# jiali-ms/JLM

Measured on AMD Instinct MI355X. Metric: decoded chars/sec at beam=10, vocab=50k (kana strings in -> n-best strings out, SURVEY 8d), higher is better.
Workload: dtype f32 (matrix products as 3-pass split-f16 MFMA, f32 accumulate; the vocabulary projection as f16 hi.hi + both cross terms in one block-scaled FP6 instruction per 32 k-values: f32-grade error, tests/test_gpu_kernels.py; scores f64; parity bars: step logits <= 1e-4 relative, 1-best identical, path scor

## Files before the change

jlm_amd/csrc/jlm_beam.hip:

```cpp
#include "jlm_common.h"
#include <type_traits>
#include <stdlib.h>

#define WL_THREADS 256
#define WL_ROWS 16

template <int MODE>
__global__ __launch_bounds__(WL_THREADS) void wordlist_kernel(
    SegTable segs, const float *__restrict__ b2, const float *__restrict__ T, int ldt,
    const int *__restrict__ g0v, const int *__restrict__ cnt, const int *__restrict__ cnt_idx,
    const int *__restrict__ wl, const int *__restrict__ wl_w, const int *__restrict__ wl_off, const int *__restrict__ wl_idx,
    int wl_base, const int *__restrict__ wl_out, float *__restrict__ edge, float *__restrict__ run_max,
    double *__restrict__ run_sum, double *__restrict__ lse, int merge, int beam) {
    extern __shared__ __attribute__((aligned(16))) float sm[];
    const int j = blockIdx.x;
    const int nrows = min(cnt[cnt_idx[j]], beam);
    if (nrows <= 0) return;
    const int gbase = g0v[j];
    const int lid = wl_base + wl_idx[j];
    const int w0 = wl_off[lid], nw = wl_off[lid + 1] - w0;
    if (MODE == 0 && nw == 0) return;
    const int tid = threadIdx.x;
    float *red = sm + (size_t)WL_ROWS * ldt;
    const int sub = tid & 7, slot = tid >> 3;
// ... 191 lines not shown
                                     int merge, int beam, int n_groups, void *stream);

extern "C" int jlm_wordlist_lse(const jlm_segment *segs_host, int n_segs, const float *b2, const float *T, int ldt,
                                const int *g0, const int *cnt, const int *cnt_idx, const int *wl, const int *wl_off,
                                const int *wl_idx, int wl_base, float *run_max, double *run_sum, double *lse, int merge,
                                int beam, int n_groups, void *stream) {
    return jlm_wordlist_lse_perm(segs_host, n_segs, b2, T, ldt, g0, cnt, cnt_idx, wl, nullptr, wl_off, wl_idx, wl_base, run_max,
                                 run_sum, lse, merge, beam, n_groups, stream);
}

extern "C" int jlm_wordlist_lse_perm(const jlm_segment *segs_host, int n_segs, const float *b2, const float *T, int ldt,
                                     const int *g0, const int *cnt, const int *cnt_idx, const int *wl, const int *wl_w,
                                     const int *wl_off, const int *wl_idx, int wl_base, float *run_max, double *run_sum,
                                     double *lse, int merge, int beam, int n_groups, void *stream) {
    SegTable t;
    if (seg_table(segs_host, n_segs, t) || ldt % 4) return -1;
    if (n_groups <= 0) return 0;
    const int form = jlm_wordlist_lse_form(segs_host, n_segs, nullptr, wl_w != nullptr, ldt, beam, 0);
    if (form < 0) return -1;
    if (form == JLM_WL_MFMA)
        return jlm_wordlist_lse_mfma(segs_host, b2, T, ldt, g0, cnt, cnt_idx, wl, wl_off, wl_idx, wl_base, run_max, run_sum,
                                     lse, merge, beam, n_groups, stream);
    const size_t lds = wl_lds_bytes(beam, ldt);
    static JlmLdsGrant grant;
    if (int rc = jlm_grant_lds(grant, reinterpret_cast<const void *>(wordlist_kernel<1>), (int)lds)) return rc;
    hipLaunchKernelGGL(wordlist_kernel<1>, dim3(n_groups), dim3(WL_THREADS), lds, (hipStream_t)stream, t, b2, T, ldt,
                       g0, cnt, cnt_idx, wl, wl_w, wl_off, wl_idx, wl_base, nullptr, nullptr, run_max, run_sum, lse, merge, beam);
    JLM_LAUNCH_CHECK();
    return 0;
}

template <int CTRL, int ROW_MASK>
__device__ __forceinline__ void argmin_dpp_step(double &v, int &i) {
    const int lo = __double2loint(v), hi = __double2hiint(v);
    const int lo2 = __builtin_amdgcn_update_dpp(lo, lo, CTRL, ROW_MASK, 0xf, false);
    const int hi2 = __builtin_amdgcn_update_dpp(hi, hi, CTRL, ROW_MASK, 0xf, false);
    const int i2 = __builtin_amdgcn_update_dpp(i, i, CTRL, ROW_MASK, 0xf, false);
    const double v2 = __hiloint2double(hi2, lo2);
    if (v2 < v || (v2 == v && i2 < i)) { v = v2; i = i2; }
}
__device__ __forceinline__ void wave_argmin(double &v, int &i) {
    argmin_dpp_step<0xB1, 0xf>(v, i);
    argmin_dpp_step<0x4E, 0xf>(v, i);
    argmin_dpp_step<0x141, 0xf>(v, i);
    argmin_dpp_step<0x140, 0xf>(v, i);
    argmin_dpp_step<0x142, 0xa>(v, i);
    argmin_dpp_step<0x143, 0xc>(v, i);
    const int lo = __builtin_amdgcn_readlane(__double2loint(v), 63);
    const int hi = __builtin_amdgcn_readlane(__double2hiint(v), 63);
    i = __builtin_amdgcn_readlane(i, 63);
    v = __hiloint2double(hi, lo);
}

template <int MODE>
__global__ __launch_bounds__(64, 8) void beam_step_kernel(jlm_lattice lat, jlm_beam_state st, int frame, int max_cands) {
    extern __shared__ __attribute__((aligned(16))) double keys[];
    const int s = blockIdx.x, lane = threadIdx.x;
    const int B = lat.n_sent, beam = lat.beam, rmax = B * beam;
    const int len = lat.sent_len[s];
    const int fs = frame * B + s;
    if (frame > len) { if (lane == 0) st.cnt[fs] = 0; return; }
    const int nb = lat.end_off[fs], ne = lat.end_off[fs + 1];
    const int gout = frame * rmax + s * beam;
    const double INF = __longlong_as_double(0x7ff0000000000000LL);
    double *Sarr = keys + max_cands;
    int *gp_of = reinterpret_cast<int *>(Sarr + (MODE == 2 ? lat.n_frames * beam : 0));
    double *lse_new = reinterpret_cast<double *>(gp_of + ((max_cands + 1) & ~1));
    int *cnt_s = reinterpret_cast<int *>(lse_new + beam);
    double *win_v = reinterpret_cast<double *>(cnt_s + ((lat.n_frames + 1) & ~1));
    int *win_i = reinterpret_cast<int *>(win_v + beam);
    int K;
    if (frame == 0) {
        K = 1;
    } else {
        const bool fused = MODE == 0 && st.lse_part != nullptr;
        const int fprev = (frame - 1) * B + s;
        for (int f = lane; f < frame; f += 64) cnt_s[f] = st.cnt[f * B + s];
        const int kprev = st.cnt[fprev];
        if (fused && kprev > 0) {
            const int base = st.live_base[fprev];
            const float2 *part = reinterpret_cast<const float2 *>(st.lse_part);
            const int sub = lane & 7;
            for (int r0 = 0; r0 < kprev; r0 += 8) {
                const int r = r0 + (lane >> 3);
                float m = JLM_NEG_BIG;
                double sm = 0.0;
                if (r < kprev)
                    for (int p = sub; p < st.n_parts; p += 8) {
                        const float2 v = part[(size_t)p * st.ld_part + base + r];
                        const float mm = fmaxf(m, v.x);
                        sm = sm * (double)expf(m - mm) + (double)v.y * (double)expf(v.x - mm);
                        m = mm;
                    }
#pragma unroll
                for (int off = 4; off >= 1; off >>= 1) {
                    const float m2 = __shfl_xor(m, off);
                    const double s2 = __shfl_xor(sm, off);
                    const float mm = fmaxf(m, m2);
                    sm = sm * (double)expf(m - mm) + s2 * (double)expf(m2 - mm);
                    m = mm;
                }
                if (sub == 0 && r < kprev) {
                    double l = (double)m + log(sm);
                    if (!(fabs(l) < 1.0e300)) { if (st.flags) atomicOr(st.flags, 1); l = 1.0e30; }
                    lse_new[r] = l;
                    st.lse[(size_t)(frame - 1) * rmax + s * beam + r] = l;
                }
            }
        }
        const int C = (ne - nb) * beam;
        if (MODE == 2) {
            for (int f = 0; f < frame; ++f) {
                const int c = st.cnt[f * B + s];
                for (int l = lane; l < c; l += 64) {
                    const int g = f * rmax + s * beam + l;
                    const int p = st.bp[g];
                    double S = 0.0;
                    if (p >= 0) {
                        const int pf = p / rmax, pk = p - pf * rmax - s * beam;
                        S = Sarr[pf * beam + pk] + st.lse[p];
                    }
                    Sarr[f * beam + l] = S;
                }
                __syncthreads();
            }
        }
        __syncthreads();
        int nvalid = 0;
        double bv = INF;
        int bi = 0x7fffffff;
        constexpr int U = 4, NREG = 8;
        double kreg[NREG];
#pragma unroll
        for (int j = 0; j < NREG; ++j) kreg[j] = INF;
        auto group = [&](int it, auto REG0) {
            constexpr int reg0 = decltype(REG0)::value;
            const int c0 = lane + 64 * U * it;
            int n[U], k[U], sf[U];
#pragma unroll
            for (int u = 0; u < U; ++u) {
                const int c = min(c0 + 64 * u, C - 1);
                n[u] = nb + c / beam;
                k[u] = c % beam;
                sf[u] = lat.node_start[n[u]];
            }
            bool ok[U];
            double scv[U], lsv[U], ysv[U];
            float ev[U];
#pragma unroll
            for (int u = 0; u < U; ++u) {
                ok[u] = (c0 + 64 * u < C) && k[u] < cnt_s[sf[u]];
                const int gp = sf[u] * rmax + s * beam + (ok[u] ? k[u] : 0);
                ev[u] = st.edge[(size_t)n[u] * beam + k[u]];
                scv[u] = (MODE == 2) ? 0.0 : st.score[gp];
                lsv[u] = (MODE == 1) ? 0.0 : st.lse[gp];
                ysv[u] = (MODE == 2) ? st.ysum[gp] : 0.0;
                if (c0 + 64 * u < C) gp_of[c0 + 64 * u] = ok[u] ? gp : -1;
            }
#pragma unroll
            for (int u = 0; u < U; ++u) {
                const int c = c0 + 64 * u;
                if (c >= C) break;
                double sc = INF;
                if (ok[u]) {
                    const double e = (double)ev[u];
                    if (MODE == 0) sc = scv[u] + (((fused && sf[u] == frame - 1) ? lse_new[k[u]] : lsv[u]) - e);
                    else if (MODE == 1) sc = scv[u] - e;
                    else sc = (Sarr[sf[u] * beam + k[u]] + lsv[u]) - (ysv[u] + e);
                    ++nvalid;
                }
                if constexpr (reg0 >= 0) kreg[reg0 + u] = sc; else keys[c] = sc;
                if (sc < bv) { bv = sc; bi = c; }
            }
        };
        group(0, std::integral_constant<int, 0>{});
        if (C > 64 * U) group(1, std::integral_constant<int, U>{});
        for (int it = 2; 64 * U * it < C; ++it) group(it, std::integral_constant<int, -1>{});
#pragma unroll
        for (int off = 32; off >= 1; off >>= 1) nvalid += __shfl_xor(nvalid, off);
        K = min(beam, nvalid);
        for (int r = 0; r < K; ++r) {
            double v = bv;
            int i = bi;
            wave_argmin(v, i);
            if (lane == 0) { win_v[r] = v; win_i[r] = i; }
            if ((i & 63) == lane) {
                const int jw = i >> 6;
                if (jw >= NREG) keys[i] = INF;
                bv = INF;
                bi = 0x7fffffff;
#pragma unroll
                for (int j = 0; j < NREG; ++j) {
                    if (j == jw) kreg[j] = INF;
                    if (kreg[j] < bv) { bv = kreg[j]; bi = lane + 64 * j; }
                }
                for (int c = lane + 64 * NREG; c < C; c += 64) {
                    const double kv = keys[c];
                    if (kv < bv) { bv = kv; bi = c; }
                }
            }
        }
        __syncthreads();
    }
    for (int r = lane; r < K; r += 64) {
        const int g = gout + r;
        if (frame == 0) {
            st.score[g] = 0.0;
            if (st.ysum) st.ysum[g] = 0.0;
            st.bp[g] = -1;
            st.node[g] = nb;
            st.word[g] = lat.node_word[nb];
        } else {
            const int wi = win_i[r];
            const int n = nb + wi / beam, k = wi % beam;
            const int gp = gp_of[wi];
            st.score[g] = win_v[r];
            if (MODE == 2) st.ysum[g] = st.ysum[gp] + (double)st.edge[(size_t)n * beam + k];
            st.bp[g] = gp;
            st.node[g] = n;
            st.word[g] = lat.node_word[n];
        }
    }
    int base = 0;
    if (lane == 0) {
        st.cnt[fs] = K;
        if (frame < len) {
            base = atomicAdd(&st.n_live[frame], K);
            if (st.live_base) st.live_base[fs] = base;
        }
    }
    base = __shfl(base, 0);
    if (frame < len)
        for (int r = lane; r < K; r += 64) st.live[(size_t)frame * rmax + base + r] = gout + r;
}

template <int MODE>
__global__ __launch_bounds__(64) void beam_step_chunked_kernel(jlm_lattice lat, jlm_beam_state st, int frame, int cap, int nch_max) {
    extern __shared__ __attribute__((aligned(16))) double keys[];
    const int s = blockIdx.x, lane = threadIdx.x;
    const int B = lat.n_sent, beam = lat.beam, rmax = B * beam;
    const int len = lat.sent_len[s];
    const int fs = frame * B + s;
    if (frame > len) { if (lane == 0) st.cnt[fs] = 0; return; }
    const int nb = lat.end_off[fs], ne = lat.end_off[fs + 1];
    const int gout = frame * rmax + s * beam;
    const double INF = __longlong_as_double(0x7ff0000000000000LL);
    double *Sarr = keys + cap;
    int *gp_of = reinterpret_cast<int *>(Sarr + (MODE == 2 ? lat.n_frames * beam : 0));
    double *lse_new = reinterpret_cast<double *>(gp_of + ((cap + 1) & ~1));
    int *cnt_s = reinterpret_cast<int *>(lse_new + beam);
    double *win_v = reinterpret_cast<double *>(cnt_s + ((lat.n_frames + 1) & ~1));
    int *win_i = reinterpret_cast<int *>(win_v + beam);
    int *win_g = win_i + beam;
    double *cw_v = reinterpret_cast<double *>(win_g + beam + (beam & 1));
    int *cw_i = reinterpret_cast<int *>(cw_v + (size_t)nch_max * beam);
    int *cw_g = cw_i + (size_t)nch_max * beam;
    int K;
    if (frame == 0) {
        K = 1;
    } else {
        const bool fused = MODE == 0 && st.lse_part != nullptr;
        const int fprev = (frame - 1) * B + s;
        for (int f = lane; f < frame; f += 64) cnt_s[f] = st.cnt[f * B + s];
        const int kprev = st.cnt[fprev];
        if (fused && kprev > 0) {
            const int base = st.live_base[fprev];
            const float2 *part = reinterpret_cast<const float2 *>(st.lse_part);
            const int sub = lane & 7;
            for (int r0 = 0; r0 < kprev; r0 += 8) {
                const int r = r0 + (lane >> 3);
                float m = JLM_NEG_BIG;
                double sm = 0.0;
                if (r < kprev)
                    for (int p = sub; p < st.n_parts; p += 8) {
                        const float2 v = part[(size_t)p * st.ld_part + base + r];
                        const float mm = fmaxf(m, v.x);
                        sm = sm * (double)expf(m - mm) + (double)v.y * (double)expf(v.x - mm);
                        m = mm;
                    }
#pragma unroll
                for (int off = 4; off >= 1; off >>= 1) {
                    const float m2 = __shfl_xor(m, off);
                    const double s2 = __shfl_xor(sm, off);
                    const float mm = fmaxf(m, m2);
                    sm = sm * (double)expf(m - mm) + s2 * (double)expf(m2 - mm);
                    m = mm;
                }
                if (sub == 0 && r < kprev) {
                    double l = (double)m + log(sm);
                    if (!(fabs(l) < 1.0e300)) { if (st.flags) atomicOr(st.flags, 1); l = 1.0e30; }
                    lse_new[r] = l;
                    st.lse[(size_t)(frame - 1) * rmax + s * beam + r] = l;
                }
            }
        }
        const int C = (ne - nb) * beam;
        if (MODE == 2) {
            for (int f = 0; f < frame; ++f) {
                const int c = st.cnt[f * B + s];
                for (int l = lane; l < c; l += 64) {
                    const int g = f * rmax + s * beam + l;
                    const int p = st.bp[g];
                    double S = 0.0;
                    if (p >= 0) {
                        const int pf = p / rmax, pk = p - pf * rmax - s * beam;
                        S = Sarr[pf * beam + pk] + st.lse[p];
                    }
                    Sarr[f * beam + l] = S;
                }
                __syncthreads();
            }
        }
        __syncthreads();
        const int nch = (C + cap - 1) / cap;
        int nvalid_all = 0;
        for (int ch = 0; ch < nch; ++ch) {
            const int c_lo = ch * cap, Cc = min(C - c_lo, cap);
            int nvalid = 0;
            double bv = INF;
            int bi = 0x7fffffff;
            for (int lc = lane; lc < Cc; lc += 64) {
                const int c = c_lo + lc;
                const int n = nb + c / beam, k = c % beam;
                const int sf = lat.node_start[n];
                const bool ok = k < cnt_s[sf];
                const int gp = sf * rmax + s * beam + (ok ? k : 0);
                double sc = INF;
                if (ok) {
                    const double e = (double)st.edge[(size_t)n * beam + k];
                    if (MODE == 0) sc = st.score[gp] + (((fused && sf == frame - 1) ? lse_new[k] : st.lse[gp]) - e);
                    else if (MODE == 1) sc = st.score[gp] - e;
                    else sc = (Sarr[sf * beam + k] + st.lse[gp]) - (st.ysum[gp] + e);
                    ++nvalid;
                }
                keys[lc] = sc;
                gp_of[lc] = ok ? gp : -1;
                if (sc < bv) { bv = sc; bi = lc; }
            }
#pragma unroll
            for (int off = 32; off >= 1; off >>= 1) nvalid += __shfl_xor(nvalid, off);
            nvalid_all += nvalid;
            const int Kc = min(beam, nvalid);
            __syncthreads();
            for (int r = 0; r < beam; ++r) {
                if (r < Kc) {
                    double v = bv;
                    int i = bi;
                    wave_argmin(v, i);
// ... 117 lines not shown
}

struct BeamStepPlan { int form, cap, nch; size_t lds; };
static BeamStepPlan beam_step_plan(int beam, int n_frames, int mode, int max_cands) {
    BeamStepPlan p = {-1, 0, 0, 0};
    if (mode < 0 || mode > 2 || beam < 1 || beam > JLM_MAX_BEAM || n_frames < 1) return p;
    if (max_cands < 1) max_cands = 1;
    const size_t lds = beam_step_lds_bytes(beam, n_frames, mode, max_cands);
    static const int chunk_env = getenv("JLM_BEAM_CHUNK") ? atoi(getenv("JLM_BEAM_CHUNK")) : 0;
    if (lds > 160 * 1024 || chunk_env > 0) {
        const int cap = chunk_env > 0 ? chunk_env : beam_step_chunk_cap(beam, n_frames, mode);
        if (cap <= 0) return p;
        const int nch = (max_cands + cap - 1) / cap;
        const size_t lds_c = beam_step_chunked_lds_bytes(beam, n_frames, mode, cap, nch);
        if (lds_c > 160 * 1024) return p;
        p.form = JLM_BEAM_STEP_CHUNKED; p.cap = cap; p.nch = nch; p.lds = lds_c;
        return p;
    }
    p.form = JLM_BEAM_STEP_ONE_PIECE; p.lds = lds;
    return p;
}

extern "C" int jlm_beam_step_form(int beam, int n_frames, int mode, int max_cands) {
    return beam_step_plan(beam, n_frames, mode, max_cands).form;
}

extern "C" int jlm_beam_step(const jlm_lattice *lat_host, const jlm_beam_state *st_host, int frame, int mode,
                             int max_cands, void *stream) {
    const jlm_lattice lat = *lat_host;
    const jlm_beam_state st = *st_host;
    if (lat.n_sent <= 0) return 0;
    if (mode == 2 && !st.ysum) return -1;
    if (mode < 0 || mode > 2) return -1;
    if (lat.beam < 1 || lat.beam > JLM_MAX_BEAM) return -1;
    if (st.lse_part && (!st.live_base || st.n_parts < 1 || mode != 0)) return -1;
    if (max_cands < 1) max_cands = 1;
    const BeamStepPlan plan = beam_step_plan(lat.beam, lat.n_frames, mode, max_cands);
    if (plan.form < 0) return -1;
    if (plan.form == JLM_BEAM_STEP_CHUNKED) {
        const int cap = plan.cap, nch = plan.nch;
        const size_t lds_c = plan.lds;
        const void *fc = mode == 0 ? (const void *)beam_step_chunked_kernel<0>
                       : mode == 1 ? (const void *)beam_step_chunked_kernel<1> : (const void *)beam_step_chunked_kernel<2>;
        static JlmLdsGrant grant_c[3];
        if (lds_c > 64 * 1024)
            if (int rc = jlm_grant_lds(grant_c[mode], fc, (int)lds_c)) return rc;
        if (mode == 0) hipLaunchKernelGGL(beam_step_chunked_kernel<0>, dim3(lat.n_sent), dim3(64), lds_c, (hipStream_t)stream, lat, st, frame, cap, nch);
        else if (mode == 1) hipLaunchKernelGGL(beam_step_chunked_kernel<1>, dim3(lat.n_sent), dim3(64), lds_c, (hipStream_t)stream, lat, st, frame, cap, nch);
        else hipLaunchKernelGGL(beam_step_chunked_kernel<2>, dim3(lat.n_sent), dim3(64), lds_c, (hipStream_t)stream, lat, st, frame, cap, nch);
        JLM_LAUNCH_CHECK();
        return 0;
    }
    const size_t lds = plan.lds;
    const void *fn = mode == 0 ? (const void *)beam_step_kernel<0>
                   : mode == 1 ? (const void *)beam_step_kernel<1> : (const void *)beam_step_kernel<2>;
    static JlmLdsGrant grant[3];
    if (lds > 64 * 1024)
        if (int rc = jlm_grant_lds(grant[mode], fn, (int)lds)) return rc;
    if (mode == 0) hipLaunchKernelGGL(beam_step_kernel<0>, dim3(lat.n_sent), dim3(64), lds, (hipStream_t)stream, lat, st, frame, max_cands);
    else if (mode == 1) hipLaunchKernelGGL(beam_step_kernel<1>, dim3(lat.n_sent), dim3(64), lds, (hipStream_t)stream, lat, st, frame, max_cands);
    else hipLaunchKernelGGL(beam_step_kernel<2>, dim3(lat.n_sent), dim3(64), lds, (hipStream_t)stream, lat, st, frame, max_cands);
    JLM_LAUNCH_CHECK();
    return 0;
}

__global__ void backtrace_kernel(jlm_lattice lat, jlm_beam_state st, int *out_nodes, int *out_len, double *out_score,
                                 int stride) {
    const int idx = blockIdx.x * blockDim.x + threadIdx.x;
    const int B = lat.n_sent, beam = lat.beam, rmax = B * beam;
    if (idx >= rmax) return;
    const int s = idx / beam, r = idx % beam;
    const int len = lat.sent_len[s];
    const int c = st.cnt[len * B + s];
    if (r >= c) { out_len[idx] = 0; out_score[idx] = 0.0; return; }
    int g = len * rmax + s * beam + r;
    out_score[idx] = st.score[g];
    int d = 0;
    while (g >= 0 && d < stride) {
        out_nodes[(size_t)idx * stride + d] = st.node[g];
        ++d;
        g = st.bp[g];
    }
    out_len[idx] = d;
}

template <int NREG>
__global__ __launch_bounds__(64) void backtrace_wave_kernel(jlm_lattice lat, jlm_beam_state st, int *out_nodes, int *out_len, double *out_score,
                                                            int stride) {
    const int s = blockIdx.x, lane = threadIdx.x;
    const int B = lat.n_sent, beam = lat.beam, rmax = B * beam;
    const int len = lat.sent_len[s];
    const int E = (len + 1) * beam;
    int nd[NREG], pl[NREG];
#pragma unroll
    for (int j = 0; j < NREG; ++j) {
        const int e = lane + 64 * j;
        const int f = e / beam, k = e - f * beam;
        const bool in = e < E;
        const size_t g = (size_t)(in ? f : 0) * rmax + s * beam + (in ? k : 0);
        const int n = st.node[g], p = st.bp[g];
        nd[j] = in ? n : -1;
        int q = -1;
        if (in && p >= 0) { const int pf = p / rmax; q = pf * beam + (p - pf * rmax - s * beam); }
        pl[j] = q;
    }
    const int c = st.cnt[len * B + s];
// ... 99 lines not shown
```

jlm_amd/csrc/jlm_gemm.hip:

```cpp
#include "jlm_common.h"

#ifdef JLM_PROFILE
static __device__ unsigned long long jlm_wg_time[4096][4];
#define JLM_WG_T(i) do { if (threadIdx.x == 0) jlm_wg_time[blockIdx.x & 4095][i] = wall_clock64(); } while (0)
extern "C" int jlm_prof_read_wg_gemm(unsigned long long *out) {
    return hipMemcpyFromSymbol(out, HIP_SYMBOL(jlm_wg_time), sizeof(jlm_wg_time)) == hipSuccess ? 0 : -1;
}
#else
#define JLM_WG_T(i) (void)0
#endif
#include <stdlib.h>

#define BK 32

template <int WM_, int WN_, int MT_, int NT_>
struct TileCfg {
    static constexpr int WAVES_M = WM_, WAVES_N = WN_, MT = MT_, NT = NT_;
    static constexpr int BM = WM_ * MT_ * 32;
    static constexpr int BN = WN_ * NT_ * 32;
    static constexpr int NTHREADS = WM_ * WN_ * 64;
};

struct PlainRows {
    const float *base;
    const int *map;
    int ld;
    int nrows;
    const int *ndev;
    struct St { const float *p; bool ok; };
    __device__ int count() const { return ndev ? min(*ndev, nrows) : nrows; }
    __device__ St init(int row, int n) const {
        St s; s.p = base; s.ok = false;
        if (row < n) {
            int r = map ? map[row] : row;
            if (r >= 0) { s.p = base + (size_t)r * ld; s.ok = true; }
        }
        return s;
    }
    __device__ const float *ptr(const St &s, int) const { return s.p; }
    __device__ bool valid(const St &s, int) const { return s.ok; }
};

struct GateRows {
    const float *h; int ldh;
    const int *rows; const int *prev; const int *word;
    const float *emb; int lde;
    int H;
    int nrows; const int *ndev;
    struct St { const float *ph; const float *pe; bool okh, oke; };
    __device__ int count() const { return ndev ? min(*ndev, nrows) : nrows; }
    __device__ St init(int row, int n) const {
        St s; s.ph = h; s.pe = emb; s.okh = false; s.oke = false;
        if (row < n) {
            int g = rows ? rows[row] : row;
            int p = prev[g];
            if (p >= 0) { s.ph = h + (size_t)p * ldh; s.okh = true; }
            s.pe = emb + (size_t)word[g] * lde;
            s.oke = true;
        }
        return s;
    }
    __device__ const float *ptr(const St &s, int k0) const { return k0 < H ? s.ph : s.pe - H; }
    __device__ bool valid(const St &s, int k0) const { return k0 < H ? s.okh : s.oke; }
};
// ... 476 lines not shown
    typename Epi::template Pre<Cfg> pre;
    epi.template prepare<Cfg>(pre, m0, M);
    float *As = smem;
    float *Bs = smem + NST * BM * 32;
    const int tid = threadIdx.x;
    const int lane = tid & 63;
    const int wave = __builtin_amdgcn_readfirstlane(tid >> 6);
    const int wm = wave / Cfg::WAVES_N, wn = wave % Cfg::WAVES_N;
    const int lrow = lane >> 3, lslot = lane & 7;
    typename ARows::St sa[L2::A_INST];
    typename BRows::St sb[L2::B_INST];
    int ka[L2::A_INST], kb[L2::B_INST];
#pragma unroll
    for (int i = 0; i < L2::A_INST; ++i) {
        const int r = (wave * L2::A_INST + i) * 8 + lrow;
        sa[i] = A.init(m0 + r, M);
        ka[i] = (lslot ^ ((r >> 1) & 7)) * 4;
    }
#pragma unroll
    for (int i = 0; i < L2::B_INST; ++i) {
        const int r = (wave * L2::B_INST + i) * 8 + lrow;
        sb[i] = B.init(n0 + r, N);
        kb[i] = (lslot ^ ((r >> 1) & 7)) * 4;
    }
    auto issue = [&](int k0, int stg) {
#pragma unroll
        for (int i = 0; i < L2::A_INST; ++i) {
            const int k = k0 + ka[i];
            const float *p = (k < K && A.valid(sa[i], k0)) ? A.ptr(sa[i], k0) + k : jlm_zero_page;
            GLDS16(p, As + (stg * BM + (wave * L2::A_INST + i) * 8) * 32);
        }
#pragma unroll
        for (int i = 0; i < L2::B_INST; ++i) {
            const int k = k0 + kb[i];
            const float *p = (k < K && B.valid(sb[i], k0)) ? B.ptr(sb[i], k0) + k : jlm_zero_page;
            GLDS16(p, Bs + (stg * BN + (wave * L2::B_INST + i) * 8) * 32);
        }
    };
    f32x16 acc[MT][NT];
#pragma unroll
    for (int mt = 0; mt < MT; ++mt)
#pragma unroll
        for (int nt = 0; nt < NT; ++nt)
#pragma unroll
            for (int r = 0; r < 16; ++r) acc[mt][nt][r] = 0.0f;
    const int nk = (K + BK - 1) / BK;
    const int li = lane & 31, h = lane >> 5;
    int goff[2][2];
#pragma unroll
    for (int st = 0; st < 2; ++st)
#pragma unroll
        for (int p = 0; p < 2; ++p) goff[st][p] = li * 32 + (((4 * st + 2 * h + p) ^ ((li >> 1) & 7)) * 4);
    JLM_WG_T(1);
#pragma unroll
    for (int q = 0; q < NST - 1; ++q)
        if (q < nk) issue(q * BK, q);
    int stg = 0;
    for (int kt = 0; kt < nk; ++kt) {
        if (kt + NST - 2 < nk) asm volatile("s_waitcnt vmcnt(%0)\n\ts_barrier" ::"n"((NST - 2) * PER) : "memory");
        else asm volatile("s_waitcnt vmcnt(0)\n\ts_barrier" ::: "memory");
        if (kt + NST - 1 < nk) issue((kt + NST - 1) * BK, stg == 0 ? NST - 1 : stg - 1);
        const float *as = As + (stg * BM + wm * MT * 32) * 32;
        const float *bs = Bs + (stg * BN + wn * NT * 32) * 32;
        f16x8 a[2][MT][2], b[2][NT][2];
#pragma unroll
        for (int st = 0; st < 2; ++st)
#pragma unroll
            for (int p = 0; p < 2; ++p) {
#pragma unroll
                for (int mt = 0; mt < MT; ++mt) a[st][mt][p] = *reinterpret_cast<const f16x8 *>(as + mt * 1024 + goff[st][p]);
#pragma unroll
                for (int nt = 0; nt < NT; ++nt) b[st][nt][p] = *reinterpret_cast<const f16x8 *>(bs + nt * 1024 + goff[st][p]);
            }
        __builtin_amdgcn_sched_barrier(0);
#pragma unroll
        for (int st = 0; st < 2; ++st)
#pragma unroll
            for (int pr = 0; pr < 3; ++pr)
#pragma unroll
                for (int mt = 0; mt < MT; ++mt)
#pragma unroll
                    for (int nt = 0; nt < NT; ++nt)
                        acc[mt][nt] = __builtin_amdgcn_mfma_f32_32x32x16_f16(a[st][mt][pr == 0 ? 1 : 0], b[st][nt][pr == 1 ? 1 : 0],
                                                                             acc[mt][nt], 0, 0, 0);
        stg = stg == NST - 1 ? 0 : stg + 1;
    }
    JLM_WG_T(2);
    __syncthreads();
    epi.template run<Cfg>(acc, m0, n0, wm, wn, lane, M, N, smem, pre);
    JLM_WG_T(3);
}

template <class Cfg, class ARows, class BRows, class Epi, int NST>
static int launch_gemm_split3(const ARows &A, const BRows &B, int K, const Epi &epi, int xcd, hipStream_t st) {
    auto kern = gemm_split3_kernel<Cfg, ARows, BRows, Epi, NST>;
    constexpr int lds = Lds2<Cfg>::BYTES / 2 * NST;
    static JlmLdsGrant grant;
    if (int rc = jlm_grant_lds(grant, reinterpret_cast<const void *>(kern), lds)) return rc;
    TileMap tm;
    tm.tiles_m = (A.nrows + Cfg::BM - 1) / Cfg::BM;
    tm.tiles_n = (B.nrows + Cfg::BN - 1) / Cfg::BN;
    tm.xcd = xcd;
    if (tm.tiles_m == 0 || tm.tiles_n == 0) return 0;
    hipLaunchKernelGGL(kern, dim3(tm.grid()), dim3(Cfg::NTHREADS), lds, st, A, B, K, epi, tm);
    JLM_LAUNCH_CHECK();
    return 0;
}

template <class Cfg, class ARows, class BRows, class Epi>
static int launch_gemm_split(const ARows &A, const BRows &B, int K, const Epi &epi, int xcd, hipStream_t st) {
    auto kern = gemm_split_kernel<Cfg, ARows, BRows, Epi>;
    constexpr int lds = Lds2<Cfg>::BYTES;
    static JlmLdsGrant grant;
    if (int rc = jlm_grant_lds(grant, reinterpret_cast<const void *>(kern), lds)) return rc;
    TileMap tm;
    tm.tiles_m = (A.nrows + Cfg::BM - 1) / Cfg::BM;
    tm.tiles_n = (B.nrows + Cfg::BN - 1) / Cfg::BN;
    tm.xcd = xcd;
    if (tm.tiles_m == 0 || tm.tiles_n == 0) return 0;
    hipLaunchKernelGGL(kern, dim3(tm.grid()), dim3(Cfg::NTHREADS), lds, st, A, B, K, epi, tm);
    JLM_LAUNCH_CHECK();
    return 0;
}

typedef TileCfg<2, 2, 2, 2> Cfg128;
typedef TileCfg<2, 2, 1, 1> Cfg64;

extern "C" int jlm_lstm_step(const float *h_in, const float *c_in, int ld_state, float *h_out, float *c_out,
                             const int *rows, const int *prev, const int *word, const float *emb, int ld_emb,
                             const float *wt, const float *bias, int kpad, int H, int E, int n_rows_max,
                             const int *n_dev, void *stream) {
    if (H % 32 != 0 || E % 4 != 0 || kpad % BK != 0 || kpad < H + E || ld_state % 4 || ld_emb % 4) return -1;
    GateRows A;
    A.h = h_in; A.ldh = ld_state; A.rows = rows; A.prev = prev; A.word = word;
    A.emb = emb; A.lde = ld_emb; A.H = H; A.nrows = n_rows_max; A.ndev = n_dev;
    PlainRows B;
    B.base = wt; B.map = nullptr; B.ld = kpad; B.nrows = 4 * H; B.ndev = nullptr;
    EpiGate epi;
    epi.c_in = c_in; epi.h_out = h_out; epi.c_out = c_out; epi.ld = ld_state;
    epi.rows = rows; epi.prev = prev; epi.bias = bias;
    const int tiles_n = 4 * H / Cfg64::BN;
    if (n_rows_max >= 8192) return launch_gemm2<TileCfg<2, 2, 2, 1>>(A, B, H + E, epi, (tiles_n % 8 == 0) ? 2 : 0, (hipStream_t)stream);
    return launch_gemm2<Cfg64>(A, B, H + E, epi, (tiles_n % 8 == 0) ? 2 : 0, (hipStream_t)stream);
}

extern "C" int jlm_gemm_nt(const float *Ap, int lda, const int *a_rows, const float *Bp, int ldb, const int *b_rows,
                           float *C, int ldc, const int *c_rows, const float *bias, int M, int N, int K,
                           const int *m_dev, void *stream) {
    if (K % 4 != 0 || lda % 4 != 0 || ldb % 4 != 0) return -1;
    PlainRows A, B;
    A.base = Ap; A.map = a_rows; A.ld = lda; A.nrows = M; A.ndev = m_dev;
    B.base = Bp; B.map = b_rows; B.ld = ldb; B.nrows = N; B.ndev = nullptr;
    EpiStore epi;
    epi.C = C; epi.c_map = c_rows; epi.ldc = ldc; epi.bias = bias;
    long tiles128 = (long)((M + 127) / 128) * ((N + 127) / 128);
    if (tiles128 < 512) return launch_gemm2<Cfg64>(A, B, K, epi, 0, (hipStream_t)stream);
    return launch_gemm2<Cfg128>(A, B, K, epi, 0, (hipStream_t)stream);
}

extern "C" int jlm_gemm_nt_split_form(int M, int N) {
    const long tiles128 = (long)((M + 127) / 128) * ((N + 127) / 128);
    const long tiles64 = (long)((M + 63) / 64) * ((N + 63) / 64);
    static int stages = -1;
    if (stages < 0) { const char *e = getenv("JLM_T_STAGES"); stages = e ? atoi(e) : 3; }
    static int txcd = -1;
    if (txcd < 0) { const char *e = getenv("JLM_T_XCD"); txcd = e ? atoi(e) : 1; }
    if (tiles64 <= 256 && stages == 3) return txcd == 0 ? JLM_T_SPLIT3_LINEAR : JLM_T_SPLIT3_XCD;
    return tiles128 < 512 ? JLM_T_CFG64 : JLM_T_CFG128;
}

extern "C" int jlm_gemm_nt_split(const void *Ap, int lda, const int *a_rows, const void *Bp, int ldb, const int *b_rows,
                                 float *C, int ldc, const int *c_rows, const float *bias, float descale, int M, int N,
                                 int K, const int *m_dev, void *stream) {
    if (K % 16 != 0 || lda % 16 != 0 || ldb % 16 != 0) return -1;
    PlainRows A, B;
    A.base = reinterpret_cast<const float *>(Ap); A.map = a_rows; A.ld = lda; A.nrows = M; A.ndev = m_dev;
    B.base = reinterpret_cast<const float *>(Bp); B.map = b_rows; B.ld = ldb; B.nrows = N; B.ndev = nullptr;
    EpiStore epi;
    epi.C = C; epi.c_map = c_rows; epi.ldc = ldc; epi.bias = bias; epi.scale = descale;
    const int form = jlm_gemm_nt_split_form(M, N);
    if (form == JLM_T_SPLIT3_LINEAR || form == JLM_T_SPLIT3_XCD)
        return launch_gemm_split3<Cfg64, PlainRows, PlainRows, EpiStore, 3>(A, B, K, epi, form == JLM_T_SPLIT3_XCD ? 1 : 0, (hipStream_t)stream);
    if (form == JLM_T_CFG64) return launch_gemm_split<Cfg64>(A, B, K, epi, 0, (hipStream_t)stream);
    return launch_gemm_split<Cfg128>(A, B, K, epi, 0, (hipStream_t)stream);
}

extern "C" int jlm_vocab_lse_partials(const float *Bseg, int ldb, int n_vocab, int K, const float *T, int ldt,
                                      const int *rows, const float *bias, float *part, int ld_part, int tile0,
                                      int n_rows_max, const int *n_dev, void *stream) {
    if (K % 4 != 0 || ldb % 4 != 0 || ldt % 4 != 0) return -1;
    PlainRows A, B;
    A.base = Bseg; A.map = nullptr; A.ld = ldb; A.nrows = n_vocab; A.ndev = nullptr;
    B.base = T; B.map = rows; B.ld = ldt; B.nrows = n_rows_max; B.ndev = n_dev;
    EpiLse epi;
    epi.bias = bias; epi.part = part; epi.ld_part = ld_part; epi.tile0 = tile0;
    int r = launch_gemm2<Cfg128>(A, B, K, epi, 1, (hipStream_t)stream);
    if (r != 0) return r > 0 ? -r : r;
    return (n_vocab + Cfg128::BM - 1) / Cfg128::BM;
}

extern "C" int jlm_vocab_lse_partials_split(const void *Bsplit, int ldb, int n_vocab, int K, const void *Tsplit, int ldt,
                                            const int *rows, const float *bias, float descale, float *part, int ld_part,
                                            int tile0, int n_rows_max, const int *n_dev, void *stream) {
    if (K % 16 != 0 || ldb % 16 != 0 || ldt % 16 != 0) return -1;
    PlainRows A, B;
    A.base = reinterpret_cast<const float *>(Bsplit); A.map = nullptr; A.ld = ldb; A.nrows = n_vocab; A.ndev = nullptr;
    B.base = reinterpret_cast<const float *>(Tsplit); B.map = rows; B.ld = ldt; B.nrows = n_rows_max; B.ndev = n_dev;
    EpiLse epi;
    epi.bias = bias; epi.part = part; epi.ld_part = ld_part; epi.tile0 = tile0; epi.scale = descale;
    int r = launch_gemm_split<Cfg128>(A, B, K, epi, 1, (hipStream_t)stream);
    if (r != 0) return r > 0 ? -r : r;
    return (n_vocab + Cfg128::BM - 1) / Cfg128::BM;
}

JLM_PROF_READER(jlm_prof_read)

template <int NK, int MT>
__device__ __forceinline__ void lse_stat_body(
    const jlm_segment &sg, const float *__restrict__ bias, int p_in_seg, int parts_in_seg, int pt, int n_paths,
    const float *__restrict__ T, int ldt, const int *__restrict__ rows, float2 *__restrict__ part_row, float *smem) {
    constexpr int BMV = 32 * MT;
    constexpr int NINST = BMV / 32;
    constexpr float LOG2E = 1.4426950408889634f, LN2 = 0.6931471805599453f;
    JLM_PROF_DECL();
    const int tid = threadIdx.x, lane = tid & 63, wave = tid >> 6;
    const int h = lane >> 5, li = lane & 31;
    const int K = sg.k, n_vocab = sg.v_end - sg.v_start, ldb = sg.ldb;
    const int ntiles = (n_vocab + BMV - 1) / BMV;
    const int vt0 = (int)((long)ntiles * p_in_seg / parts_in_seg), vt1 = (int)((long)ntiles * (p_in_seg + 1) / parts_in_seg);
    const float *__restrict__ Bp = sg.B;
    const int prow = pt * 128 + wave * 32 + li;
    const bool row_ok = prow < n_paths;
    const float *trow = T + (size_t)(row_ok ? (rows ? rows[prow] : prow) : 0) * ldt + sg.t_off;
    const int nq_last = (K - 32 * (NK - 1) + 7) >> 3;
    f32x4 tf[NK][4];
// ... 433 lines not shown
```

Before: 3.037 million.

## Software-pipeline split3 GEMM with 4 stages and restructure beam step loads

The split3 GEMM moves to a 4-stage ring. LDS fragment reads for the next k-step are double-buffered in registers and interleaved between the two MFMA halves of the current step, so LDS latency overlaps compute. In the beam step kernel, the LSE partial fold is factored into a helper that handles two rows per pass and batches several loads before the exp math. Candidate scoring is split into dependent load levels using 32-bit byte offsets and scalar-hinted header loads, and MODE 0 widens the first group to 8 candidates. This adds register pressure and LDS, and adds a size guard for the 32-bit offsets.

After: 3.127 million (median of 6 runs). 2.9% higher.

```diff
diff --git a/jlm_amd/csrc/jlm_beam.hip b/jlm_amd/csrc/jlm_beam.hip
--- a/jlm_amd/csrc/jlm_beam.hip
+++ b/jlm_amd/csrc/jlm_beam.hip
@@ -267,15 +267,83 @@
     v = __hiloint2double(hi, lo);
 }
 
+#define BEAM_FOLD_NB 4
+__device__ __forceinline__ void beam_fold_parts(const jlm_beam_state &st, int lane, int kprev, int base, double *lse_new,
+                                                double *lse_out) {
+    const float2 *part = reinterpret_cast<const float2 *>(st.lse_part);
+    const int sub = lane & 7, n_parts = st.n_parts;
+    for (int r0 = 0; r0 < kprev; r0 += 16) {
+        int r[2];
+        const float2 *row[2];
+        float m[2];
+        double sm[2];
+#pragma unroll
+        for (int h = 0; h < 2; ++h) {
+            r[h] = r0 + 8 * h + (lane >> 3);
+            row[h] = part + base + min(r[h], kprev - 1);
+            m[h] = JLM_NEG_BIG;
+            sm[h] = 0.0;
+        }
+        for (int pb = 0; pb < n_parts; pb += 8 * BEAM_FOLD_NB) {
+            float2 v[2][BEAM_FOLD_NB];
+#pragma unroll
+            for (int h = 0; h < 2; ++h)
+#pragma unroll
+                for (int j = 0; j < BEAM_FOLD_NB; ++j) v[h][j] = row[h][(size_t)min(pb + sub + 8 * j, n_parts - 1) * st.ld_part];
+            __builtin_amdgcn_sched_barrier(0);
+#pragma unroll
+            for (int h = 0; h < 2; ++h)
+#pragma unroll
+                for (int j = 0; j < BEAM_FOLD_NB; ++j)
+                    if (r[h] < kprev && pb + sub + 8 * j < n_parts) {
+                        const float mm = fmaxf(m[h], v[h][j].x);
+                        sm[h] = fma(sm[h], (double)expf(m[h] - mm), __dmul_rn((double)v[h][j].y, (double)expf(v[h][j].x - mm)));
+                        m[h] = mm;
+                    }
+            __builtin_amdgcn_s_waitcnt(0x0F70);
+        }
+#pragma unroll
+        for (int h = 0; h < 2; ++h) {
+            if (r0 + 8 * h >= kprev) break;
+            float mh = m[h];
+            double sh = sm[h];
+#pragma unroll
+            for (int off = 4; off >= 1; off >>= 1) {
+                const float m2 = __shfl_xor(mh, off);
+                const double s2 = __shfl_xor(sh, off);
+                const float mm = fmaxf(mh, m2);
+                sh = fma(sh, (double)expf(mh - mm), __dmul_rn(s2, (double)expf(m2 - mm)));
+                mh = mm;
+            }
+            if (sub == 0 && r[h] < kprev) {
+                double l = (double)mh + log(sh);
+                if (!(fabs(l) < 1.0e300)) { if (st.flags) atomicOr(st.flags, 1); l = 1.0e30; }
+                lse_new[r[h]] = l;
+                lse_out[r[h]] = l;
+            }
+        }
+    }
+}
+
+template <class T>
+__device__ __forceinline__ T beam_ld(const T *base, unsigned byte_off) {
+    return *reinterpret_cast<const T *>(reinterpret_cast<const char *>(base) + byte_off);
+}
+
 template <int MODE>
 __global__ __launch_bounds__(64, 8) void beam_step_kernel(jlm_lattice lat, jlm_beam_state st, int frame, int max_cands) {
     extern __shared__ __attribute__((aligned(16))) double keys[];
     const int s = blockIdx.x, lane = threadIdx.x;
     const int B = lat.n_sent, beam = lat.beam, rmax = B * beam;
-    const int len = lat.sent_len[s];
     const int fs = frame * B + s;
+    const bool fused = MODE == 0 && st.lse_part != nullptr;
+    const int fprev = frame > 0 ? fs - B : fs;
+    const int *lbase = fused ? st.live_base : st.cnt;
+    int len = lat.sent_len[s];
+    int nb = lat.end_off[fs], ne = lat.end_off[fs + 1];
+    int kprev = st.cnt[fprev], pbase = lbase[fprev];
+    asm volatile("" : "+s"(len), "+s"(nb), "+s"(ne), "+s"(kprev), "+s"(pbase));
     if (frame > len) { if (lane == 0) st.cnt[fs] = 0; return; }
-    const int nb = lat.end_off[fs], ne = lat.end_off[fs + 1];
     const int gout = frame * rmax + s * beam;
     const double INF = __longlong_as_double(0x7ff0000000000000LL);
     double *Sarr = keys + max_cands;
@@ -288,41 +356,10 @@
     if (frame == 0) {
         K = 1;
     } else {
-        const bool fused = MODE == 0 && st.lse_part != nullptr;
-        const int fprev = (frame - 1) * B + s;
-        for (int f = lane; f < frame; f += 64) cnt_s[f] = st.cnt[f * B + s];
-        const int kprev = st.cnt[fprev];
-        if (fused && kprev > 0) {
-            const int base = st.live_base[fprev];
-            const float2 *part = reinterpret_cast<const float2 *>(st.lse_part);
-            const int sub = lane & 7;
-            for (int r0 = 0; r0 < kprev; r0 += 8) {
-                const int r = r0 + (lane >> 3);
-                float m = JLM_NEG_BIG;
-                double sm = 0.0;
-                if (r < kprev)
-                    for (int p = sub; p < st.n_parts; p += 8) {
-                        const float2 v = part[(size_t)p * st.ld_part + base + r];
-                        const float mm = fmaxf(m, v.x);
-                        sm = sm * (double)expf(m - mm) + (double)v.y * (double)expf(v.x - mm);
-                        m = mm;
-                    }
-#pragma unroll
-                for (int off = 4; off >= 1; off >>= 1) {
-                    const float m2 = __shfl_xor(m, off);
-                    const double s2 = __shfl_xor(sm, off);
-                    const float mm = fmaxf(m, m2);
-                    sm = sm * (double)expf(m - mm) + s2 * (double)expf(m2 - mm);
-                    m = mm;
-                }
-                if (sub == 0 && r < kprev) {
-                    double l = (double)m + log(sm);
-                    if (!(fabs(l) < 1.0e300)) { if (st.flags) atomicOr(st.flags, 1); l = 1.0e30; }
-                    lse_new[r] = l;
-                    st.lse[(size_t)(frame - 1) * rmax + s * beam + r] = l;
-                }
-            }
-        }
+        const int cnt_lane = st.cnt[min(lane, frame - 1) * B + s];
+        if (fused && kprev > 0) beam_fold_parts(st, lane, kprev, pbase, lse_new, st.lse + ((size_t)(frame - 1) * rmax + s * beam));
+        if (lane < frame) cnt_s[lane] = cnt_lane;
+        for (int f = lane + 64; f < frame; f += 64) cnt_s[f] = st.cnt[f * B + s];
         const int C = (ne - nb) * beam;
         if (MODE == 2) {
             for (int f = 0; f < frame; ++f) {
@@ -348,49 +385,87 @@
         double kreg[NREG];
 #pragma unroll
         for (int j = 0; j < NREG; ++j) kreg[j] = INF;
-        auto group = [&](int it, auto REG0) {
+        const int gprev = (frame - 1) * rmax + s * beam;
+        const int *cell_start = lat.node_start + nb;
+        const float *cell_edge = st.edge + (size_t)nb * beam;
+        auto level1 = [&](int it, auto NCc, int *k, int *sf, float *ev) {
+            constexpr int NC = decltype(NCc)::value;
+            const int c0 = lane + 64 * U * it;
+#pragma unroll
+            for (int j = 0; j < NC; ++j) {
+                const int c = min(c0 + 64 * j, C - 1);
+                const int q = (int)((unsigned)c / (unsigned)beam);
+                k[j] = c - q * beam;
+                sf[j] = beam_ld(cell_start, (unsigned)q * 4u);
+                ev[j] = beam_ld(cell_edge, (unsigned)c * 4u);
+            }
+        };
+        auto level2 = [&](int it, auto NCc, const int *k, int *sf, double *scv, double *lsv, double *ysv) -> unsigned {
+            constexpr int NC = decltype(NCc)::value;
+            const int c0 = lane + 64 * U * it;
+            unsigned okm = 0;
+#pragma unroll
+            for (int j = 0; j < NC; ++j) {
+                const bool live = k[j] < cnt_s[sf[j]], ok = live & (c0 + 64 * j < C);
+                const int gp = sf[j] * rmax + s * beam + (live ? k[j] : 0);
+                scv[j] = (MODE == 2) ? 0.0 : beam_ld(st.score, (unsigned)gp * 8u);
+                lsv[j] = (MODE == 1) ? 0.0 : beam_ld(st.lse, (unsigned)gp * 8u);
+                ysv[j] = (MODE == 2) ? beam_ld(st.ysum, (unsigned)gp * 8u) : 0.0;
+                gp_of[min(c0 + 64 * j, C - 1)] = live ? gp : -1;
+                okm |= (ok ? 1u : 0u) << j;
+                sf[j] = (MODE == 2) ? sf[j] * beam + k[j] : -1;
+            }
+            return okm;
+        };
+        auto finish = [&](int it, auto NCc, auto REG0, unsigned okm, const int *sel, const float *ev, const double *scv,
+                          const double *lsv, const double *ysv) {
+            constexpr int NC = decltype(NCc)::value;
             constexpr int reg0 = decltype(REG0)::value;
             const int c0 = lane + 64 * U * it;
-            int n[U], k[U], sf[U];
-#pragma unroll
-            for (int u = 0; u < U; ++u) {
-                const int c = min(c0 + 64 * u, C - 1);
-                n[u] = nb + c / beam;
-                k[u] = c % beam;
-                sf[u] = lat.node_start[n[u]];
-            }
-            bool ok[U];
-            double scv[U], lsv[U], ysv[U];
-            float ev[U];
-#pragma unroll
-            for (int u = 0; u < U; ++u) {
-                ok[u] = (c0 + 64 * u < C) && k[u] < cnt_s[sf[u]];
-                const int gp = sf[u] * rmax + s * beam + (ok[u] ? k[u] : 0);
-                ev[u] = st.edge[(size_t)n[u] * beam + k[u]];
-                scv[u] = (MODE == 2) ? 0.0 : st.score[gp];
-                lsv[u] = (MODE == 1) ? 0.0 : st.lse[gp];
-                ysv[u] = (MODE == 2) ? st.ysum[gp] : 0.0;
-                if (c0 + 64 * u < C) gp_of[c0 + 64 * u] = ok[u] ? gp : -1;
-            }
-#pragma unroll
-            for (int u = 0; u < U; ++u) {
-                const int c = c0 + 64 * u;
-                if (c >= C) break;
-                double sc = INF;
-                if (ok[u]) {
-                    const double e = (double)ev[u];
-                    if (MODE == 0) sc = scv[u] + (((fused && sf[u] == frame - 1) ? lse_new[k[u]] : lsv[u]) - e);
-                    else if (MODE == 1) sc = scv[u] - e;
-                    else sc = (Sarr[sf[u] * beam + k[u]] + lsv[u]) - (ysv[u] + e);
-                    ++nvalid;
-                }
-                if constexpr (reg0 >= 0) kreg[reg0 + u] = sc; else keys[c] = sc;
+#pragma unroll
+            for (int j = 0; j < NC; ++j) {
+                const int c = c0 + 64 * j;
+                const bool ok = (okm >> j) & 1u;
+                const double e = (double)ev[j];
+                double t;
+                if (MODE == 0) {
+                    const int kp = gp_of[min(c, C - 1)] - gprev;
+                    const bool from_fold = fused && (unsigned)kp < (unsigned)beam;
+                    double ln = lse_new[from_fold ? kp : 0];
+                    asm volatile("" : "+v"(ln));
+                    t = scv[j] + ((from_fold ? ln : lsv[j]) - e);
+                } else if (MODE == 1) {
+                    t = scv[j] - e;
+                } else {
+                    t = (Sarr[sel[j]] + lsv[j]) - (ysv[j] + e);
+                }
+                const double sc = ok ? t : INF;
+                nvalid += ok ? 1 : 0;
+                if constexpr (reg0 >= 0) kreg[reg0 + j] = sc; else if (c < C) keys[c] = sc;
                 if (sc < bv) { bv = sc; bi = c; }
             }
         };
-        group(0, std::integral_constant<int, 0>{});
-        if (C > 64 * U) group(1, std::integral_constant<int, U>{});
-        for (int it = 2; 64 * U * it < C; ++it) group(it, std::integral_constant<int, -1>{});
+        auto take = [&](int it, auto NCc, auto REG0) {
+            constexpr int NC = decltype(NCc)::value;
+            int k[NC], sf[NC];
+            float ev[NC];
+            double scv[NC], lsv[NC], ysv[NC];
+            level1(it, NCc, k, sf, ev);
+            const unsigned okm = level2(it, NCc, k, sf, scv, lsv, ysv);
+            finish(it, NCc, REG0, okm, sf, ev, scv, lsv, ysv);
+        };
+        using I0 = std::integral_constant<int, 0>;
+        using IU = std::integral_constant<int, U>;
+        using IR = std::integral_constant<int, NREG>;
+        using IL = std::integral_constant<int, -1>;
+        if constexpr (MODE == 0) {
+            take(0, IR{}, I0{});
+            for (int it = 2; 64 * U * it < C; ++it) take(it, IU{}, IL{});
+        } else {
+            take(0, IU{}, I0{});
+            if (C > 64 * U) take(1, IU{}, IU{});
+            for (int it = 2; 64 * U * it < C; ++it) take(it, IU{}, IL{});
+        }
 #pragma unroll
         for (int off = 32; off >= 1; off >>= 1) nvalid += __shfl_xor(nvalid, off);
         K = min(beam, nvalid);
@@ -478,37 +553,8 @@
         const int fprev = (frame - 1) * B + s;
         for (int f = lane; f < frame; f += 64) cnt_s[f] = st.cnt[f * B + s];
         const int kprev = st.cnt[fprev];
-        if (fused && kprev > 0) {
-            const int base = st.live_base[fprev];
-            const float2 *part = reinterpret_cast<const float2 *>(st.lse_part);
-            const int sub = lane & 7;
-            for (int r0 = 0; r0 < kprev; r0 += 8) {
-                const int r = r0 + (lane >> 3);
-                float m = JLM_NEG_BIG;
-                double sm = 0.0;
-                if (r < kprev)
-                    for (int p = sub; p < st.n_parts; p += 8) {
-                        const float2 v = part[(size_t)p * st.ld_part + base + r];
-                        const float mm = fmaxf(m, v.x);
-                        sm = sm * (double)expf(m - mm) + (double)v.y * (double)expf(v.x - mm);
-                        m = mm;
-                    }
-#pragma unroll
-                for (int off = 4; off >= 1; off >>= 1) {
-                    const float m2 = __shfl_xor(m, off);
-                    const double s2 = __shfl_xor(sm, off);
-                    const float mm = fmaxf(m, m2);
-                    sm = sm * (double)expf(m - mm) + s2 * (double)expf(m2 - mm);
-                    m = mm;
-                }
-                if (sub == 0 && r < kprev) {
-                    double l = (double)m + log(sm);
-                    if (!(fabs(l) < 1.0e300)) { if (st.flags) atomicOr(st.flags, 1); l = 1.0e30; }
-                    lse_new[r] = l;
-                    st.lse[(size_t)(frame - 1) * rmax + s * beam + r] = l;
-                }
-            }
-        }
+        if (fused && kprev > 0)
+            beam_fold_parts(st, lane, kprev, st.live_base[fprev], lse_new, st.lse + ((size_t)(frame - 1) * rmax + s * beam));
         const int C = (ne - nb) * beam;
         if (MODE == 2) {
             for (int f = 0; f < frame; ++f) {
@@ -732,6 +778,7 @@
         return 0;
     }
     const size_t lds = plan.lds;
+    if ((size_t)lat.n_frames * lat.n_sent * lat.beam > ((size_t)1 << 29)) return -1;
     const void *fn = mode == 0 ? (const void *)beam_step_kernel<0>
                    : mode == 1 ? (const void *)beam_step_kernel<1> : (const void *)beam_step_kernel<2>;
     static JlmLdsGrant grant[3];
diff --git a/jlm_amd/csrc/jlm_gemm.hip b/jlm_amd/csrc/jlm_gemm.hip
--- a/jlm_amd/csrc/jlm_gemm.hip
+++ b/jlm_amd/csrc/jlm_gemm.hip
@@ -10,6 +10,7 @@
 #define JLM_WG_T(i) (void)0
 #endif
 #include <stdlib.h>
+#include <type_traits>
 
 #define BK 32
 
@@ -592,39 +593,60 @@
 #pragma unroll
         for (int p = 0; p < 2; ++p) goff[st][p] = li * 32 + (((4 * st + 2 * h + p) ^ ((li >> 1) & 7)) * 4);
     JLM_WG_T(1);
+    static_assert(NST == 4, "the loop below refills the stage of step kt - 1 with step kt + 3");
 #pragma unroll
     for (int q = 0; q < NST - 1; ++q)
         if (q < nk) issue(q * BK, q);
-    int stg = 0;
-    for (int kt = 0; kt < nk; ++kt) {
-        if (kt + NST - 2 < nk) asm volatile("s_waitcnt vmcnt(%0)\n\ts_barrier" ::"n"((NST - 2) * PER) : "memory");
-        else asm volatile("s_waitcnt vmcnt(0)\n\ts_barrier" ::: "memory");
-        if (kt + NST - 1 < nk) issue((kt + NST - 1) * BK, stg == 0 ? NST - 1 : stg - 1);
+    f16x8 a[2][2][MT][2], b[2][2][NT][2];
+    auto read = [&](auto SET, int stg) {
+        constexpr int set = decltype(SET)::value;
         const float *as = As + (stg * BM + wm * MT * 32) * 32;
         const float *bs = Bs + (stg * BN + wn * NT * 32) * 32;
-        f16x8 a[2][MT][2], b[2][NT][2];
 #pragma unroll
         for (int st = 0; st < 2; ++st)
 #pragma unroll
             for (int p = 0; p < 2; ++p) {
 #pragma unroll
-                for (int mt = 0; mt < MT; ++mt) a[st][mt][p] = *reinterpret_cast<const f16x8 *>(as + mt * 1024 + goff[st][p]);
-#pragma unroll
-                for (int nt = 0; nt < NT; ++nt) b[st][nt][p] = *reinterpret_cast<const f16x8 *>(bs + nt * 1024 + goff[st][p]);
-            }
+                for (int mt = 0; mt < MT; ++mt) a[set][st][mt][p] = *reinterpret_cast<const f16x8 *>(as + mt * 1024 + goff[st][p]);
+#pragma unroll
+                for (int nt = 0; nt < NT; ++nt) b[set][st][nt][p] = *reinterpret_cast<const f16x8 *>(bs + nt * 1024 + goff[st][p]);
+            }
+    };
+    auto mfmas = [&](auto SET, int st) {
+        constexpr int set = decltype(SET)::value;
+#pragma unroll
+        for (int pr = 0; pr < 3; ++pr)
+#pragma unroll
+            for (int mt = 0; mt < MT; ++mt)
+#pragma unroll
+                for (int nt = 0; nt < NT; ++nt)
+                    acc[mt][nt] = __builtin_amdgcn_mfma_f32_32x32x16_f16(a[set][st][mt][pr == 0 ? 1 : 0], b[set][st][nt][pr == 1 ? 1 : 0],
+                                                                         acc[mt][nt], 0, 0, 0);
+    };
+    auto step = [&](int kt, auto CUR, auto NXT) {
+        if (kt + 1 < nk) {
+            if (kt + 2 < nk) asm volatile("s_waitcnt vmcnt(%0)\n\ts_barrier" ::"n"(PER) : "memory");
+            else asm volatile("s_waitcnt vmcnt(0)\n\ts_barrier" ::: "memory");
+        }
         __builtin_amdgcn_sched_barrier(0);
-#pragma unroll
-        for (int st = 0; st < 2; ++st)
-#pragma unroll
-            for (int pr = 0; pr < 3; ++pr)
-#pragma unroll
-                for (int mt = 0; mt < MT; ++mt)
-#pragma unroll
-                    for (int nt = 0; nt < NT; ++nt)
-                        acc[mt][nt] = __builtin_amdgcn_mfma_f32_32x32x16_f16(a[st][mt][pr == 0 ? 1 : 0], b[st][nt][pr == 1 ? 1 : 0],
-                                                                             acc[mt][nt], 0, 0, 0);
-        stg = stg == NST - 1 ? 0 : stg + 1;
-    }
+        mfmas(CUR, 0);
+        __builtin_amdgcn_sched_barrier(0);
+        read(NXT, (kt + 1) & (NST - 1));
+        if (kt + 3 < nk) issue((kt + 3) * BK, (kt + 3) & (NST - 1));
+        __builtin_amdgcn_sched_barrier(0);
+        mfmas(CUR, 1);
+    };
+    if (nk >= 3) asm volatile("s_waitcnt vmcnt(%0)\n\ts_barrier" ::"n"(2 * PER) : "memory");
+    else if (nk == 2) asm volatile("s_waitcnt vmcnt(%0)\n\ts_barrier" ::"n"(PER) : "memory");
+    else asm volatile("s_waitcnt vmcnt(0)\n\ts_barrier" ::: "memory");
+    using S0 = std::integral_constant<int, 0>;
+    using S1 = std::integral_constant<int, 1>;
+    if (nk > 0) read(S0{}, 0);
+    for (int kt = 0; kt + 1 < nk; kt += 2) {
+        step(kt, S0{}, S1{});
+        step(kt + 1, S1{}, S0{});
+    }
+    if (nk & 1) step(nk - 1, S0{}, S1{});
     JLM_WG_T(2);
     __syncthreads();
     epi.template run<Cfg>(acc, m0, n0, wm, wn, lane, M, N, smem, pre);
@@ -720,7 +742,7 @@
     epi.C = C; epi.c_map = c_rows; epi.ldc = ldc; epi.bias = bias; epi.scale = descale;
     const int form = jlm_gemm_nt_split_form(M, N);
     if (form == JLM_T_SPLIT3_LINEAR || form == JLM_T_SPLIT3_XCD)
-        return launch_gemm_split3<Cfg64, PlainRows, PlainRows, EpiStore, 3>(A, B, K, epi, form == JLM_T_SPLIT3_XCD ? 1 : 0, (hipStream_t)stream);
+        return launch_gemm_split3<Cfg64, PlainRows, PlainRows, EpiStore, 4>(A, B, K, epi, form == JLM_T_SPLIT3_XCD ? 1 : 0, (hipStream_t)stream);
     if (form == JLM_T_CFG64) return launch_gemm_split<Cfg64>(A, B, K, epi, 0, (hipStream_t)stream);
     return launch_gemm_split<Cfg128>(A, B, K, epi, 0, (hipStream_t)stream);
 }
```
